# dmMaze/comic-text-detector

Measured on NVIDIA H100. Metric: pages/sec @1024x1024 synthetic, higher is better.
Workload: dtype fp16

## Files before the change

comic-text-detector_b200/csrc/refine_mk.cu:

```cuda
#include <cuda_runtime.h>
#include <limits.h>
#include <math.h>

#include "kernels.h"

namespace ctd {

namespace {

constexpr int kThreads = 256;
constexpr int kChunkPx = kRefineChunkPx;

struct WinState {
  int hist[4][256];
  unsigned long long xs[12];
  int lo[3], hi[3], otsu_t[3], ncol;
  int nproc, proc_kind[4], proc_neg[4];
  int area0, max1, cnt1, max2;
  int pad[2];
};

struct Ctx {
  const uint8_t* img_all;
  const uint8_t* mask_all;
  uint32_t* out_all;
  const RefineWin* wins;
  const RefineChunk* chunks;
  WinState* st;
  int mode;
  uint16_t* lab;
  uint16_t* roots;
  int* nroots;
  int* P;
  int* acc;
  uint8_t* grey;
  unsigned* cand;
  unsigned *pred, *merged, *tmp;
  size_t plane_words;
};
constexpr uint16_t kNoLabel = 0xffffu;
constexpr unsigned kMergeBit = 0x8000u;
static_assert(kChunkPx <= int(kMergeBit), "a chunk-local offset fits the 15 bits below kMergeBit");

struct View {
  RefineWin win;
  int w, rw, rh, y0, x0, rows, cols, i0, cnt, woff;
  const uint8_t* img;
  const uint8_t* mask;
};

__device__ __forceinline__ View view_of(const Ctx& c, int chunk) {
  View v;
  const RefineChunk ch = c.chunks[chunk];
  v.w = ch.win;
  v.win = c.wins[ch.win];
  v.rw = v.win.x2 - v.win.x1;
  v.rh = v.win.y2 - v.win.y1;
  v.y0 = ch.y0;
  v.x0 = ch.x0;
  v.rows = ch.rows;
  v.cols = min(v.rw - ch.x0, kChunkPx);
  v.i0 = ch.y0 * v.rw + ch.x0;
  v.cnt = ch.rows * v.cols;
  v.woff = ch.woff;
  v.img = c.img_all + size_t(v.win.page_off) * 3;
  v.mask = c.mask_all + size_t(v.win.page_off);
  return v;
}

__device__ __forceinline__ int chunk_start(int y, int x, int rw) {
  if (rw > kChunkPx) return y * rw + (x & ~(kChunkPx - 1));
  const int rows_per = refine_rows_per_chunk(rw);
  return (y / rows_per) * rows_per * rw;
}
static_assert((kChunkPx & (kChunkPx - 1)) == 0, "row segments start on multiples of kChunkPx");

__device__ __forceinline__ int uf_find(const int* L, int a) {
  int p = __ldcg(L + a);
  while (p != a) {
    a = p;
    p = __ldcg(L + a);
  }
  return a;
}
__device__ __forceinline__ int uf_find_compress(int* L, int a) {
  const int r = uf_find(L, a);
  while (a != r) {
    const int p = __ldcg(L + a);
    if (p <= r) break;
    atomicMin(&L[a], r);
    a = p;
  }
  return r;
}
__device__ __forceinline__ void uf_union(int* L, int a, int b) {
  bool done;
  do {
    a = uf_find(L, a);
    b = uf_find(L, b);
    if (a < b) {
      const int old = atomicMin(&L[b], a);
      done = old == b;
      b = old;
    } else if (b < a) {
      const int old = atomicMin(&L[a], b);
      done = old == a;
      a = old;
    } else {
      done = true;
    }
  } while (!done);
}

__device__ __forceinline__ void hist_add(int* hist, int bin) {
  const int b0 = __shfl_sync(0xffffffffu, bin, 0);
  if (__all_sync(0xffffffffu, bin == b0)) {
    if ((threadIdx.x & 31) == 0 && bin >= 0) atomicAdd(&hist[bin], 32);
    return;
  }
  if (bin >= 0) atomicAdd(&hist[bin], 1);
}

struct DivW { int d; float inv; bool fast; };
__device__ __forceinline__ DivW make_div(int d, int n) { return DivW{d, __frcp_rn(float(d)), n < (1 << 24)}; }
__device__ __forceinline__ void divmod(int i, const DivW& dv, int& q, int& r) {
  if (dv.fast) {
    q = __float2int_rz(__int2float_rn(i) * dv.inv);
    r = i - q * dv.d;
    if (r < 0) { --q; r += dv.d; } else if (r >= dv.d) { ++q; r -= dv.d; }
  } else {
    q = i / dv.d;
    r = i - q * dv.d;
  }
}

__device__ __forceinline__ unsigned tail_mask(int w, int cnt) {
  const int rem = cnt - 32 * w;
  return rem >= 32 ? 0xffffffffu : (1u << rem) - 1u;
}
__device__ __forceinline__ unsigned row_start_bits(int x0, int rw) {
  unsigned rs = 0u;
  for (int j = x0 == 0 ? 0 : rw - x0; j < 32; j += rw) rs |= 1u << j;
  return rs;
}
__device__ __forceinline__ int run_end(unsigned M, unsigned S, int sbit) {
  const unsigned stop = (~M | S) & (0xfffffffeu << sbit);
  return stop ? __ffs(stop) - 2 : 31;
}
__device__ __forceinline__ unsigned span_bits(int lo, int hi) {
  return (hi == 31 ? 0xffffffffu : ((2u << hi) - 1u)) & ~((1u << lo) - 1u);
}
__device__ __forceinline__ unsigned copied_word(const unsigned* src, int sb, int len, int db, int d) {
  const int r = 32 * d - db;
  if (r <= -32 || r >= len) return 0u;
  const int pos = sb + max(r, 0);
  unsigned o = __funnelshift_r(src[pos >> 5], src[(pos >> 5) + 1], pos & 31);
  if (len - max(r, 0) < 32) o &= (1u << (len - max(r, 0))) - 1u;
  return r < 0 ? o << -r : o;
}

constexpr int kU = 4;
constexpr int kExtWords = (3 * kChunkPx) / 32 + 4;
static_assert(3 * (kChunkPx + 2) / 32 + 2 < kExtWords, "a row segment's halo rectangle fits the shared bit masks");
struct Halo {
  int ystart, xs, ew, ext, off;
};
__device__ __forceinline__ Halo halo_of(const View& v) {
  Halo h;
  h.ystart = v.y0 > 0 ? v.y0 - 1 : 0;
  h.xs = v.x0 > 0 ? v.x0 - 1 : 0;
  h.ew = min(v.x0 + v.cols + 1, v.rw) - h.xs;
  h.ext = (min(v.y0 + v.rows + 1, v.rh) - h.ystart) * h.ew;
  h.off = (v.y0 - h.ystart) * h.ew + v.x0 - h.xs;
  return h;
}
__device__ __forceinline__ unsigned bits_from(const unsigned* M, int pos) {
  if (pos <= -32) return 0u;
  if (pos < 0) return M[0] << (-pos);
  const int w = pos >> 5, sft = pos & 31;
  return __funnelshift_r(M[w], M[w + 1], sft);
}
__device__ __forceinline__ void row_ends(int x, int rw, unsigned& rs, unsigned& re) {
  rs = row_start_bits(x, rw);
  int xe = x + 32;
  if (xe >= rw) xe %= rw;
  re = (rs >> 1) | (xe == 0 ? 0x80000000u : 0u);
}
__global__ void __launch_bounds__(kThreads) k_phase0(Ctx c) {
  __shared__ int sh[4][256];
  __shared__ unsigned N60[kExtWords], N127[kExtWords];
  __shared__ unsigned F127[kChunkPx / 32 + 1];
  const View v = view_of(c, blockIdx.x);
  for (int i = threadIdx.x; i < 1024; i += kThreads) (&sh[0][0])[i] = 0;
  for (int i = threadIdx.x; i < kExtWords; i += kThreads) { N60[i] = 0u; N127[i] = 0u; }
  __syncthreads();
  uint8_t* grey = c.grey + v.win.off;
  const Halo hl = halo_of(v);
  const DivW dv = make_div(hl.ew, 3 * (kChunkPx + 2) + 1);
  for (int e0 = 0; e0 < hl.ext; e0 += kThreads) {
    const int e = e0 + threadIdx.x;
    int mv = 255;
    if (e < hl.ext) {
      int ye, xe;
      divmod(e, dv, ye, xe);
      mv = v.mask[size_t(v.win.y1 + hl.ystart + ye) * v.win.pitch + v.win.x1 + hl.xs + xe];
    }
    const unsigned b60 = __ballot_sync(0xffffffffu, mv <= 60), b127 = __ballot_sync(0xffffffffu, mv <= 127);
    if ((threadIdx.x & 31) == 0 && e < hl.ext) { N60[e >> 5] = b60; N127[e >> 5] = b127; }
  }
  __syncthreads();
  const int ew = hl.ew;
  for (int w = threadIdx.x; w * 32 < v.cnt; w += kThreads) {
    const int p = w * 32 + hl.off;
    int ye, xe;
    divmod(p, dv, ye, xe);
    unsigned rs, re;
    row_ends(hl.xs + xe, v.rw, rs, re);
    const unsigned f60 = bits_from(N60, p) | bits_from(N60, p - ew) | bits_from(N60, p + ew) | (bits_from(N60, p - 1) & ~rs) |
                         (bits_from(N60, p + 1) & ~re);
    c.pred[v.woff + w] = ~f60 & tail_mask(w, v.cnt);
    c.merged[v.woff + w] = 0u;
    F127[w] = bits_from(N127, p) | bits_from(N127, p - ew) | bits_from(N127, p + ew) |
              ((bits_from(N127, p - 1) | bits_from(N127, p - ew - 1) | bits_from(N127, p + ew - 1)) & ~rs) |
              ((bits_from(N127, p + 1) | bits_from(N127, p - ew + 1) | bits_from(N127, p + ew + 1)) & ~re);
  }
  __syncthreads();
  const DivW dvw = make_div(v.rw, v.rw * v.rh);
  for (int k0 = 0; k0 < v.cnt; k0 += kThreads * kU) {
    int b[kU], g[kU], r[kU];
#pragma unroll
    for (int u = 0; u < kU; ++u) {
      const int k = k0 + u * kThreads + threadIdx.x;
      b[u] = -1; g[u] = -1; r[u] = -1;
      if (k < v.cnt) {
        int y, x;
        divmod(v.i0 + k, dvw, y, x);
        const size_t gp = size_t(v.win.y1 + y) * v.win.pitch + v.win.x1 + x;
        b[u] = v.img[gp * 3]; g[u] = v.img[gp * 3 + 1]; r[u] = v.img[gp * 3 + 2];
      }
    }
#pragma unroll
    for (int u = 0; u < kU; ++u) {
      const int k = k0 + u * kThreads + threadIdx.x;
      const bool in = k < v.cnt;
      int gr = 0;
      bool core = false;
      if (in) {
        const int i = v.i0 + k;
        gr = (b[u] * 1868 + g[u] * 9617 + r[u] * 4899 + 8192) >> 14;
        grey[i] = (uint8_t)gr;
        core = !((F127[k >> 5] >> (k & 31)) & 1u);
      }
      if (k0 + u * kThreads < v.cnt) {
        hist_add(sh[1], b[u]);
        hist_add(sh[2], g[u]);
        hist_add(sh[3], r[u]);
        hist_add(sh[0], core ? gr : -1);
      }
    }
  }
  __syncthreads();
  int* gh = &c.st[v.w].hist[0][0];
  for (int i = threadIdx.x; i < 1024; i += kThreads) {
    const int val = (&sh[0][0])[i];
    if (val) atomicAdd(&gh[i], val);
  }
}

constexpr int kDecideThreads = 64;
__global__ void __launch_bounds__(kDecideThreads) k_decide1(Ctx c) {
  __shared__ int cnt255[256];
  __shared__ int order[256];
  __shared__ double edges[256];
  __shared__ int s_first, s_last, s_total;
  __shared__ int hist_s[4][256];
  WinState& st = c.st[blockIdx.x];
  const RefineWin win = c.wins[blockIdx.x];
  const int n = (win.x2 - win.x1) * (win.y2 - win.y1);
  for (int i = threadIdx.x; i < 1024; i += kDecideThreads) (&hist_s[0][0])[i] = (&st.hist[0][0])[i];
  const int* hist_g = hist_s[0];
  for (int i = threadIdx.x; i < 256; i += kDecideThreads) cnt255[i] = 0;
  __syncthreads();
  if (threadIdx.x == 0) {
    int first = -1, last = -1, total = 0;
    for (int v = 0; v < 256; ++v)
      if (hist_g[v]) { if (first < 0) first = v; last = v; total += hist_g[v]; }
    s_first = first; s_last = last; s_total = total;
  }
  __syncthreads();
  {
    double fe, le;
    if (s_total == 0) { fe = 0.0; le = 1.0; }
    else if (s_first == s_last) { fe = s_first - 0.5; le = s_last + 0.5; }
    else { fe = s_first; le = s_last; }
    const double step = (le - fe) / 255.0;
    for (int i = threadIdx.x; i < 256; i += kDecideThreads) edges[i] = (i == 255) ? le : __dadd_rn(__dmul_rn((double)i, step), fe);
    __syncthreads();
    for (int v = threadIdx.x; v < 256; v += kDecideThreads) {
      if (!hist_g[v]) continue;
      const double a = (double)v;
      const double f = ((a - fe) / (le - fe)) * 255.0;
      int idx = (int)f;
      if (idx == 255) idx = 254;
      if (a < edges[idx]) --idx;
      if (a >= edges[idx + 1] && idx != 254) ++idx;
      atomicAdd(&cnt255[idx], hist_g[v]);
    }
  }
  __syncthreads();
  for (int b = threadIdx.x; b < 255; b += kDecideThreads) {
    int rank = 0;
    const int cb = cnt255[b];
    for (int q = 0; q < 255; ++q) rank += (cnt255[q] > cb) || (cnt255[q] == cb && q < b);
    order[rank] = b;
  }
  __syncthreads();
  if (threadIdx.x == 0) {
    double top[3];
    int nt = 1;
    top[0] = edges[order[0]];
    const double tol = (double)s_total * 0.001;
    for (int j = 1; j < 255; ++j) {
      const double col = edges[order[j]];
      double dmin = 1e300;
      for (int t = 0; t < nt; ++t) dmin = fmin(dmin, fabs(top[t] - col));
      if (dmin > 10.0) top[nt++] = col;
      if (nt >= 3 || (double)cnt255[order[j]] < tol) break;
    }
    st.ncol = nt;
    for (int t = 0; t < nt; ++t) {
      const double c_top = fmin(top[t] + 30.0, 255.0);
      const double c_bot = c_top - 60.0;
      st.lo[t] = (int)fmin(fmax(rint(c_bot), 0.0), 255.0);
      st.hi[t] = (int)fmin(fmax(rint(c_top), 0.0), 255.0);
    }
  }
  if (threadIdx.x >= 32 && threadIdx.x < 35) {
    const int* hh = hist_s[1 + threadIdx.x - 32];
    const double scale = 1.0 / (double)n;
    double mu = 0;
    for (int i = 0; i < 256; ++i) mu = __dadd_rn(mu, __dmul_rn((double)i, (double)hh[i]));
    mu = __dmul_rn(mu, scale);
    double mu1 = 0, q1 = 0, max_sigma = 0;
    int max_val = 0;
    for (int i = 0; i < 256; ++i) {
      const double p_i = __dmul_rn((double)hh[i], scale);
      mu1 = __dmul_rn(mu1, q1);
      q1 = __dadd_rn(q1, p_i);
      const double q2 = 1.0 - q1;
      if (fmin(q1, q2) < 1.1920929e-07 || fmax(q1, q2) > 1.0 - 1.1920929e-07) continue;
      mu1 = __ddiv_rn(__dadd_rn(mu1, __dmul_rn((double)i, p_i)), q1);
      const double mu2 = __ddiv_rn(__dsub_rn(mu, __dmul_rn(q1, mu1)), q2);
      const double dm = __dsub_rn(mu1, mu2);
      const double sigma = __dmul_rn(__dmul_rn(__dmul_rn(q1, q2), dm), dm);
      if (sigma > max_sigma) { max_sigma = sigma; max_val = i; }
    }
    st.otsu_t[threadIdx.x - 32] = max_val;
  }
}

__global__ void __launch_bounds__(kThreads) k_xor(Ctx c) {
  __shared__ unsigned long long sx[12];
  __shared__ unsigned Cw[6][kChunkPx / 32];
  const View v = view_of(c, blockIdx.x);
  const WinState& st = c.st[v.w];
  if (threadIdx.x < 12) sx[threadIdx.x] = 0ull;
  __syncthreads();
  const uint8_t* grey = c.grey + v.win.off;
  const int ncol = st.ncol;
  int lo[3], hi[3], ot[3];
#pragma unroll
  for (int k = 0; k < 3; ++k) { lo[k] = st.lo[k]; hi[k] = st.hi[k]; ot[k] = st.otsu_t[k]; }
  unsigned pos[6], npx = 0;
#pragma unroll
  for (int k = 0; k < 6; ++k) pos[k] = 0u;
  const DivW dv = make_div(v.rw, v.rw * v.rh);
  for (int k0 = 0; k0 < v.cnt; k0 += kThreads * kU) {
    int mk[kU], gr[kU], ch[kU][3];
#pragma unroll
    for (int u = 0; u < kU; ++u) {
      const int k = k0 + u * kThreads + threadIdx.x;
      mk[u] = -1; gr[u] = 0;
#pragma unroll
      for (int q = 0; q < 3; ++q) ch[u][q] = 0;
      if (k < v.cnt) {
        int y, x;
        divmod(v.i0 + k, dv, y, x);
        const size_t gp = size_t(v.win.y1 + y) * v.win.pitch + v.win.x1 + x;
        mk[u] = v.mask[gp];
        gr[u] = grey[v.i0 + k];
#pragma unroll
        for (int q = 0; q < 3; ++q) ch[u][q] = v.img[gp * 3 + q];
      }
    }
#pragma unroll
    for (int u = 0; u < kU; ++u) {
      const int kb = k0 + u * kThreads + (int(threadIdx.x) & ~31);
      if (kb >= v.cnt) continue;
      const bool in = mk[u] >= 0;
      npx += in;
#pragma unroll
      for (int k = 0; k < 3; ++k) {
        const bool t = in && gr[u] >= lo[k] && gr[u] <= hi[k];
        const bool t2 = in && ch[u][k] > ot[k];
        if (in) {
          pos[k] += (unsigned)((t ? 255 : 0) ^ mk[u]);
          pos[3 + k] += (unsigned)((t2 ? 255 : 0) ^ mk[u]);
        }
        const unsigned b = __ballot_sync(0xffffffffu, t), b2 = __ballot_sync(0xffffffffu, t2);
        if ((threadIdx.x & 31) == 0) { Cw[k][kb >> 5] = b; Cw[3 + k][kb >> 5] = b2; }
      }
    }
  }
#pragma unroll
  for (int k = 0; k < 6; ++k) {
    const bool used = k >= 3 || k < ncol;
    unsigned long long sp = used ? pos[k] : 0ull, sn = used ? 255ull * npx - pos[k] : 0ull;
    for (int o = 16; o > 0; o >>= 1) {
      sp += __shfl_down_sync(0xffffffffu, sp, o);
      sn += __shfl_down_sync(0xffffffffu, sn, o);
    }
    if ((threadIdx.x & 31) == 0) {
      if (sp) atomicAdd(&sx[2 * k], sp);
      if (sn) atomicAdd(&sx[2 * k + 1], sn);
    }
  }
  __syncthreads();
  if (threadIdx.x < 12 && sx[threadIdx.x]) atomicAdd(&c.st[v.w].xs[threadIdx.x], sx[threadIdx.x]);
  const int nw = (v.cnt + 31) >> 5;
  for (int k = 0; k < 6; ++k) {
    if (k < 3 && k >= ncol) continue;
    unsigned* cw = c.cand + k * c.plane_words + v.woff;
    for (int w = threadIdx.x; w < nw; w += kThreads) cw[w] = Cw[k][w];
  }
}

__global__ void k_decide2(Ctx c, int n_wins) {
  const int w = blockIdx.x * blockDim.x + threadIdx.x;
  if (w >= n_wins) return;
  WinState& st = c.st[w];
  const unsigned long long* xs = st.xs;
  unsigned long long best[4];
  int kind[4], neg[4], np_ = 0;
  for (int k = 0; k < st.ncol; ++k) {
    const bool ng = xs[2 * k + 1] < xs[2 * k];
    best[np_] = ng ? xs[2 * k + 1] : xs[2 * k];
    kind[np_] = k; neg[np_] = ng; ++np_;
  }
  int bc = 0, bneg = 0;
  unsigned long long bv = ~0ull;
  for (int ch = 0; ch < 3; ++ch) {
    const bool ng = xs[6 + 2 * ch + 1] < xs[6 + 2 * ch];
    const unsigned long long val = ng ? xs[6 + 2 * ch + 1] : xs[6 + 2 * ch];
    if (val < bv) { bv = val; bc = ch; bneg = ng; }
  }
  best[np_] = bv; kind[np_] = 3 + bc; neg[np_] = bneg; ++np_;
  for (int i = 1; i < np_; ++i) {
    const unsigned long long val = best[i];
    const int kk = kind[i], nn = neg[i];
    int j = i - 1;
    while (j >= 0 && best[j] > val) { best[j + 1] = best[j]; kind[j + 1] = kind[j]; neg[j + 1] = neg[j]; --j; }
    best[j + 1] = val; kind[j + 1] = kk; neg[j + 1] = nn;
  }
  for (int i = 0; i < np_; ++i) { st.proc_kind[i] = kind[i]; st.proc_neg[i] = neg[i]; }
  st.nproc = np_;
  st.area0 = 0; st.max1 = -1; st.cnt1 = 0; st.max2 = -1;
}

constexpr int kLabelThreads = 512;

struct Source { const unsigned* words; unsigned flip; };
__device__ __forceinline__ Source source_of(const Ctx& c, const WinState& st, const View& v, int round) {
  if (round == 4) return Source{c.merged + v.woff, 0xffffffffu};
  return Source{c.cand + size_t(st.proc_kind[round]) * c.plane_words + v.woff, st.proc_neg[round] ? 0xffffffffu : 0u};
}

__device__ void apply_merges(const Ctx& c, const View& v, int chunk, int round, unsigned* dec) {
  for (int i = threadIdx.x; i < kChunkPx / 32; i += blockDim.x) dec[i] = 0u;
  __syncthreads();
  const uint16_t* roots = c.roots + v.win.off + v.i0;
  const int nr = c.nroots[chunk];
  bool any = false;
  for (int j = threadIdx.x; j < nr; j += blockDim.x) {
    const unsigned e = roots[j];
    if (e & kMergeBit) { atomicOr(&dec[(e ^ kMergeBit) >> 5], 1u << (e & 31)); any = true; }
  }
  if (!__syncthreads_or(any)) return;
  const uint16_t* lab = c.lab + v.win.off + v.i0;
  const Source src = source_of(c, c.st[v.w], v, round);
  unsigned* merged = c.merged + v.woff;
  const DivW dv = make_div(v.rw, kChunkPx + 1);
  for (int hw0 = 0; hw0 * 16 < v.cnt; hw0 += blockDim.x) {
    const int hw = hw0 + threadIdx.x, w = hw >> 1;
    unsigned add = 0u;
    if (hw * 16 < v.cnt) {
      const unsigned M = (src.words[w] ^ src.flip) & tail_mask(w, v.cnt);
      if (M) {
        int yl, x0;
        divmod(w * 32, dv, yl, x0);
        const unsigned S = M & (~(M << 1) | row_start_bits(x0, v.rw));
        for (unsigned f = S & ((hw & 1) ? 0xffff0000u : 0x0000ffffu); f; f &= f - 1u) {
          const int sbit = __ffs(f) - 1;
          const unsigned l = lab[w * 32 + sbit];
          if ((dec[l >> 5] >> (l & 31)) & 1u) add |= span_bits(sbit, run_end(M, S, sbit));
        }
      }
    }
    add |= __shfl_xor_sync(0xffffffffu, add, 1);
    if (add && !(hw & 1)) merged[w] |= add;
  }
  __syncthreads();
}

__device__ __forceinline__ int suf_find(const int* L, int a) {
  int p = L[a];
  while (p != a) {
    a = p;
    p = L[a];
  }
  return a;
}
__device__ __forceinline__ int suf_find_halve(int* L, int a) {
  int p = L[a];
  while (p != a) {
    const int gp = L[p];
    if (gp != p) atomicMin(&L[a], gp);
    a = p;
    p = gp;
  }
  return a;
}
__device__ __forceinline__ void suf_union(int* L, int a, int b) {
  bool done;
  do {
    a = suf_find_halve(L, a);
    b = suf_find_halve(L, b);
    if (a < b) {
      const int old = atomicMin(&L[b], a);
      done = old == b;
      b = old;
    } else if (b < a) {
      const int old = atomicMin(&L[a], b);
      done = old == a;
      a = old;
    } else {
      done = true;
    }
  } while (!done);
}

#ifdef CTD_REFINE_PASS_CLOCKS
__device__ unsigned long long g_pass_clocks[5][8];
#define PASS_CLOCK_BEGIN() long long pass_t0 = clock64()
#define PASS_CLOCK(pass)                                                                        \
  do {                                                                                          \
    __syncthreads();                                                                            \
    if (threadIdx.x == 0) {                                                                     \
      const long long t = clock64();                                                            \
      atomicAdd(&g_pass_clocks[round][pass], (unsigned long long)(t - pass_t0));                \
      pass_t0 = t;                                                                              \
    }                                                                                           \
  } while (0)
#else
#define PASS_CLOCK_BEGIN()
#define PASS_CLOCK(pass)
#endif

__global__ void __launch_bounds__(kLabelThreads, 3) k_label_local(Ctx c, int round) {
  __shared__ int Ls[kChunkPx];
  __shared__ unsigned Mw[kChunkPx / 32 + 2];
  __shared__ unsigned Sw[kChunkPx / 32];
  __shared__ unsigned Gw[kChunkPx / 32];
  __shared__ unsigned Bw[kChunkPx / 32];
  __shared__ int s_fg, s_nroot;
  const View v = view_of(c, blockIdx.x);
  WinState& st = c.st[v.w];
  PASS_CLOCK_BEGIN();
  if (round >= 1 && round <= 3 && round - 1 < st.nproc) apply_merges(c, v, blockIdx.x, round - 1, Sw);
  if (round < 4 && round >= st.nproc) return;
  PASS_CLOCK(0);
  for (int i = threadIdx.x; i < kChunkPx / 32 + 2; i += kLabelThreads) Mw[i] = 0u;
  if (threadIdx.x == 0) { s_fg = 0; s_nroot = 0; }
  __syncthreads();
  uint16_t* lab = c.lab + v.win.off + v.i0;
  uint16_t* roots = c.roots + v.win.off + v.i0;
  int* P = c.P + v.win.off;
  int* acc = c.acc + 4 * v.win.off;
  const int n = v.rw * v.rh;
  int* area = acc; int* gain = acc + n; int* loss = acc + 2 * n; int* maxi = acc + 3 * n;
  const DivW dv = make_div(v.rw, kChunkPx + 1);
  {
    const Source src = source_of(c, st, v, round);
    const unsigned* mgw = c.merged + v.woff;
    const unsigned* pdw = c.pred + v.woff;
    for (int hw = threadIdx.x; hw * 16 < v.cnt; hw += kLabelThreads) {
      const int w = hw >> 1;
      const unsigned M = (src.words[w] ^ src.flip) & tail_mask(w, v.cnt);
      int yl, x0;
      divmod(w * 32, dv, yl, x0);
      const unsigned S = M & (~(M << 1) | row_start_bits(x0, v.rw));
      if (!(hw & 1)) {
        const unsigned un = M & ~mgw[w], pd = pdw[w];
        Mw[w] = M; Sw[w] = S; Gw[w] = un & pd; Bw[w] = un & ~pd;
      }
      for (unsigned f = S & ((hw & 1) ? 0xffff0000u : 0x0000ffffu); f; f &= f - 1u) {
        const int k = w * 32 + __ffs(f) - 1;
        Ls[k] = k;
      }
    }
  }
  __syncthreads();
  PASS_CLOCK(1);
  auto start_of = [&](int pos) -> int {
    return (pos & ~31) + 31 - __clz(Sw[pos >> 5] & (0xffffffffu >> (31 - (pos & 31))));
  };
  auto bits_at = [&](int pos) -> unsigned {
    if (pos <= -32) return 0u;
    if (pos < 0) return Mw[0] << (-pos);
    const int w = pos >> 5, sft = pos & 31;
    return __funnelshift_r(Mw[w], Mw[w + 1], sft);
  };
  for (int hw = threadIdx.x; hw * 16 < v.cnt; hw += kLabelThreads) {
    const int w = hw >> 1;
    const unsigned half = (hw & 1) ? 0xffff0000u : 0x0000ffffu;
    const unsigned cur = Mw[w];
    if (!(cur & half)) continue;
    const int k0 = w * 32;
    int yl, x0;
    divmod(k0, dv, yl, x0);
    const unsigned rs = row_start_bits(x0, v.rw);
    int xe = x0 + 32;
    if (xe >= v.rw) xe %= v.rw;
    const unsigned re = (rs >> 1) | (xe == 0 ? 0x80000000u : 0u);
    const unsigned lft = bits_at(k0 - 1);
    if (!(hw & 1) && (cur & 1u) && !(rs & 1u) && (lft & 1u)) suf_union(Ls, k0, start_of(k0 - 1));
    if (k0 + 32 <= v.rw) continue;
    const unsigned vup = (k0 >= v.rw ? 0xffffffffu : (0xffffffffu << (v.rw - k0))) & half;
    const unsigned up = bits_at(k0 - v.rw), upl = bits_at(k0 - v.rw - 1), upr = bits_at(k0 - v.rw + 1);
    unsigned f = cur & up & vup & (rs | ~lft | ~upl);
    while (f) {
      const int j = __ffs(f) - 1;
      f &= f - 1u;
      suf_union(Ls, start_of(k0 + j), start_of(k0 + j - v.rw));
    }
    const unsigned nb = cur & ~up & vup;
    f = nb & upl & ~rs;
    while (f) {
      const int j = __ffs(f) - 1;
      f &= f - 1u;
      suf_union(Ls, start_of(k0 + j), start_of(k0 + j - v.rw - 1));
    }
    f = nb & upr & ~re;
    while (f) {
      const int j = __ffs(f) - 1;
      f &= f - 1u;
      suf_union(Ls, start_of(k0 + j), start_of(k0 + j - v.rw + 1));
    }
  }
  __syncthreads();
  PASS_CLOCK(3);
  int fgc = 0;
  for (int hw = threadIdx.x; hw * 16 < v.cnt; hw += kLabelThreads) {
    const unsigned half = (hw & 1) ? 0xffff0000u : 0x0000ffffu;
    unsigned f = Sw[hw >> 1] & half;
    fgc += __popc(Mw[hw >> 1] & half);
    const int k0 = (hw >> 1) * 32;
    while (f) {
      const int s0 = k0 + __ffs(f) - 1;
      f &= f - 1u;
      const int r = suf_find(Ls, s0);
      if (r != s0) {
        atomicMin(&Ls[s0], r);
      } else {
        const int gi = v.i0 + s0;
        area[gi] = 0; gain[gi] = 0; loss[gi] = 0; maxi[gi] = -1;
        P[gi] = gi;
        roots[atomicAdd(&s_nroot, 1)] = uint16_t(s0);
      }
    }
  }
  if (round == 4) {
    for (int o = 16; o > 0; o >>= 1) fgc += __shfl_down_sync(0xffffffffu, fgc, o);
    if ((threadIdx.x & 31) == 0 && fgc) atomicAdd(&s_fg, fgc);
  }
  __syncthreads();
  if (threadIdx.x == 0) {
    c.nroots[blockIdx.x] = s_nroot;
    const int a0 = v.cnt - s_fg;
    if (round == 4 && a0) atomicAdd(&st.area0, a0);
  }
  PASS_CLOCK(4);
  for (int k = threadIdx.x; k < v.cnt; k += kLabelThreads)
    lab[k] = ((Mw[k >> 5] >> (k & 31)) & 1u) ? uint16_t(Ls[start_of(k)]) : kNoLabel;
  PASS_CLOCK(5);
  for (int hw = threadIdx.x; hw * 16 < v.cnt; hw += kLabelThreads) {
    const int w = hw >> 1;
    const unsigned M = Mw[w], S = Sw[w];
    unsigned f = S & ((hw & 1) ? 0xffff0000u : 0x0000ffffu);
    if (!f) continue;
    const unsigned G = Gw[w], B = Bw[w];
    const int k0 = w * 32;
    while (f) {
      const int sbit = __ffs(f) - 1;
      f &= f - 1u;
      const int e = run_end(M, S, sbit);
      const unsigned rm = span_bits(sbit, e);
      const int gi = v.i0 + Ls[k0 + sbit];
      atomicAdd(&area[gi], __popc(rm));
      atomicMax(&maxi[gi], v.i0 + k0 + e);
      const int g_ = __popc(rm & G), l_ = __popc(rm & B);
      if (g_) atomicAdd(&gain[gi], g_);
      if (l_) atomicAdd(&loss[gi], l_);
    }
  }
  PASS_CLOCK(6);
}
constexpr int kBorderThreads = 256;
__global__ void __launch_bounds__(kBorderThreads) k_union_border(Ctx c, int round) {
  const View v = view_of(c, blockIdx.x);
  if (round < 4 && round >= c.st[v.w].nproc) return;
  if (v.i0 == 0) return;
  const uint16_t* lab = c.lab + v.win.off;
  int* P = c.P + v.win.off;
  auto root_at = [&](int y, int x) { const int i = y * v.rw + x; return chunk_start(y, x, v.rw) + lab[i]; };
  const int y = v.y0;
  if (v.x0 > 0 && threadIdx.x == 0 && lab[v.i0] != kNoLabel && lab[v.i0 - 1] != kNoLabel)
    uf_union(P, v.i0 + lab[v.i0], root_at(y, v.x0 - 1));
  if (y == 0) return;
  for (int k = threadIdx.x; k < v.cols; k += int(blockDim.x)) {
    const int i = v.i0 + k, x = v.x0 + k;
    if (lab[i] == kNoLabel) continue;
    const int up = i - v.rw;
    const int r = v.i0 + lab[i];
    if (lab[up] != kNoLabel) {
      const bool first = x == 0 || lab[i - 1] == kNoLabel || lab[up - 1] == kNoLabel;
      if (first) uf_union(P, r, root_at(y - 1, x));
    } else {
      if (x > 0 && lab[up - 1] != kNoLabel) uf_union(P, r, root_at(y - 1, x - 1));
      if (x + 1 < v.rw && lab[up + 1] != kNoLabel) uf_union(P, r, root_at(y - 1, x + 1));
    }
  }
}
__global__ void __launch_bounds__(kThreads) k_flat1(Ctx c, int round) {
  const View v = view_of(c, blockIdx.x);
  if (round < 4 && round >= c.st[v.w].nproc) return;
  const uint16_t* roots = c.roots + v.win.off + v.i0;
  const int nr = c.nroots[blockIdx.x];
  int* P = c.P + v.win.off;
  int* acc = c.acc + 4 * v.win.off;
  const int n = v.rw * v.rh;
  int* area = acc; int* gain = acc + n; int* loss = acc + 2 * n; int* maxi = acc + 3 * n;
  for (int j = threadIdx.x; j < nr; j += kThreads) {
    const int cr = v.i0 + roots[j];
    const int g = uf_find_compress(P, cr);
    if (g != cr) {
      atomicAdd(&area[g], area[cr]);
      atomicMax(&maxi[g], maxi[cr]);
      const int g_ = gain[cr], l_ = loss[cr];
      if (g_) atomicAdd(&gain[g], g_);
      if (l_) atomicAdd(&loss[g], l_);
    }
  }
}
__global__ void __launch_bounds__(kThreads) k_top_a(Ctx c) {
  const View v = view_of(c, blockIdx.x);
  WinState& st = c.st[v.w];
  const int* P = c.P + v.win.off;
  const int* area = c.acc + 4 * v.win.off;
  const uint16_t* roots = c.roots + v.win.off + v.i0;
  const int nr = c.nroots[blockIdx.x];
  int m = -1;
  for (int j = threadIdx.x; j < nr; j += kThreads) {
    const int i = v.i0 + roots[j];
    if (P[i] == i) m = max(m, area[i]);
  }
  if (v.i0 == 0 && threadIdx.x == 0) m = max(m, st.area0);
  for (int o = 16; o > 0; o >>= 1) m = max(m, __shfl_down_sync(0xffffffffu, m, o));
  if ((threadIdx.x & 31) == 0 && m >= 0) atomicMax(&st.max1, m);
}
__global__ void __launch_bounds__(kThreads) k_top_b(Ctx c) {
  const View v = view_of(c, blockIdx.x);
  WinState& st = c.st[v.w];
  const int* P = c.P + v.win.off;
  const int* area = c.acc + 4 * v.win.off;
  const uint16_t* roots = c.roots + v.win.off + v.i0;
  const int nr = c.nroots[blockIdx.x];
  const int m1 = st.max1;
  int m2 = -1, c1 = 0;
  auto push = [&](int a) { if (a == m1) ++c1; else m2 = max(m2, a); };
  for (int j = threadIdx.x; j < nr; j += kThreads) {
    const int i = v.i0 + roots[j];
    if (P[i] == i) push(area[i]);
  }
  if (v.i0 == 0 && threadIdx.x == 0) push(st.area0);
  for (int o = 16; o > 0; o >>= 1) {
    m2 = max(m2, __shfl_down_sync(0xffffffffu, m2, o));
    c1 += __shfl_down_sync(0xffffffffu, c1, o);
  }
  if ((threadIdx.x & 31) == 0) {
    if (c1) atomicAdd(&st.cnt1, c1);
    if (m2 >= 0) atomicMax(&st.max2, m2);
  }
}
__global__ void __launch_bounds__(kThreads) k_decide_roots(Ctx c, int round) {
  const View v = view_of(c, blockIdx.x);
  const WinState& st = c.st[v.w];
  if (round < 4 && round >= st.nproc) return;
  const int* P = c.P + v.win.off;
  const int* acc = c.acc + 4 * v.win.off;
  const int n = v.rw * v.rh;
  const int* area = acc; const int* gain = acc + n; const int* loss = acc + 2 * n; const int* maxi = acc + 3 * n;
  const int second = st.cnt1 >= 2 ? st.max1 : st.max2;
  const int thresh = second >= 0 ? second : st.max1;
  uint16_t* roots = c.roots + v.win.off + v.i0;
  const int nr = c.nroots[blockIdx.x];
  for (int j = threadIdx.x; j < nr; j += kThreads) {
    const int cl = roots[j];
    const int g = P[v.i0 + cl];
    const int a = area[g];
    bool ok;
    if (round < 4) {
      const int mx = maxi[g];
      ok = !(a == 1 || (a == 2 && (mx == g + 1 || mx == g + v.rw)));
    } else {
      ok = a < thresh;
    }
    if (ok && gain[g] > loss[g]) roots[j] = uint16_t(cl | kMergeBit);
  }
}
__global__ void __launch_bounds__(kThreads) k_merge(Ctx c, int round) {
  __shared__ unsigned dec[kChunkPx / 32];
  const View v = view_of(c, blockIdx.x);
  if (round >= c.st[v.w].nproc) return;
  apply_merges(c, v, blockIdx.x, round, dec);
}

__global__ void __launch_bounds__(kThreads) k_dilate(Ctx c) {
  __shared__ unsigned Mw[kExtWords];
  const View v = view_of(c, blockIdx.x);
  for (int i = threadIdx.x; i < kExtWords; i += kThreads) Mw[i] = 0u;
  __syncthreads();
  const Halo hl = halo_of(v);
  const int ew = hl.ew;
  const DivW dv = make_div(ew, 3 * (kChunkPx + 2) + 1);
  const bool seg = v.rw > kChunkPx;
  const int nseg = (v.rw + kChunkPx - 1) / kChunkPx;
  const int rows_up = seg ? 1 : refine_rows_per_chunk(v.rw);
  if (!seg) {
    const bool up = v.y0 > 0, down = v.y0 + v.rows < v.rh;
    const unsigned* mu = up ? c.merged + c.chunks[blockIdx.x - 1].woff : nullptr;
    const unsigned* md = down ? c.merged + c.chunks[blockIdx.x + 1].woff : nullptr;
    for (int d = threadIdx.x; d * 32 < hl.ext; d += kThreads) {
      unsigned m = copied_word(c.merged + v.woff, 0, v.cnt, hl.off, d);
      if (up) m |= copied_word(mu, (rows_up - 1) * v.rw, v.rw, 0, d);
      if (down) m |= copied_word(md, 0, v.rw, hl.off + v.cnt, d);
      Mw[d] = m;
    }
  }
  for (int e0 = 0; seg && e0 < hl.ext; e0 += kThreads) {
    const int e = e0 + threadIdx.x;
    bool bit = false;
    if (e < hl.ext) {
      int ye, xe;
      divmod(e, dv, ye, xe);
      const int y = hl.ystart + ye, x = hl.xs + xe;
      const int dy = y < v.y0 ? -1 : (y >= v.y0 + v.rows ? 1 : 0);
      int ch = int(blockIdx.x) + dy * (seg ? nseg : 1), k;
      if (seg) {
        ch += x / kChunkPx - v.x0 / kChunkPx;
        k = x % kChunkPx;
      } else {
        k = (dy < 0 ? rows_up - 1 : (dy > 0 ? 0 : y - v.y0)) * v.rw + x;
      }
      const int wo = ch == int(blockIdx.x) ? v.woff : c.chunks[ch].woff;
      bit = (c.merged[wo + (k >> 5)] >> (k & 31)) & 1u;
    }
    const unsigned m = __ballot_sync(0xffffffffu, bit);
    if ((threadIdx.x & 31) == 0 && e < hl.ext) Mw[e >> 5] = m;
  }
  __syncthreads();
  for (int w = threadIdx.x; w * 32 < v.cnt; w += kThreads) {
    const int p = w * 32 + hl.off;
    int ye, xe;
    divmod(p, dv, ye, xe);
    unsigned rs, re;
    row_ends(hl.xs + xe, v.rw, rs, re);
    unsigned o = bits_from(Mw, p) | bits_from(Mw, p - ew) | bits_from(Mw, p + ew);
    o |= (bits_from(Mw, p - 1) | bits_from(Mw, p - ew - 1) | bits_from(Mw, p + ew - 1)) & ~rs;
    o |= (bits_from(Mw, p + 1) | bits_from(Mw, p - ew + 1) | bits_from(Mw, p + ew + 1)) & ~re;
    c.tmp[v.woff + w] = o & tail_mask(w, v.cnt);
  }
}
__global__ void __launch_bounds__(kThreads) k_or(Ctx c) {
  __shared__ unsigned dec[kChunkPx / 32];
  const View v = view_of(c, blockIdx.x);
  apply_merges(c, v, blockIdx.x, 4, dec);
  const unsigned* merged = c.merged + v.woff;
  const DivW dv = make_div(v.rw, v.rw * v.rh);
  for (int k = threadIdx.x; k < v.cnt; k += kThreads) {
    if (!((merged[k >> 5] >> (k & 31)) & 1u)) continue;
    int y, x;
    divmod(v.i0 + k, dv, y, x);
    const size_t gp = size_t(v.win.page_off) + size_t(v.win.y1 + y) * v.win.pitch + v.win.x1 + x;
    atomicOr(&c.out_all[gp >> 2], 0xffu << (8 * (gp & 3)));
  }
}

}

#ifdef CTD_REFINE_PASS_CLOCKS
extern "C" __attribute__((visibility("default"))) int ctd_refine_pass_clocks(unsigned long long* out) {
  static const unsigned long long zero[5 * 8] = {};
  cudaError_t e = cudaMemcpyFromSymbol(out, g_pass_clocks, sizeof(zero));
  if (e == cudaSuccess) e = cudaMemcpyToSymbol(g_pass_clocks, zero, sizeof(zero));
  return int(e);
}
#endif

size_t refine_mk_state_bytes(int n_wins) { return (size_t(n_wins) * sizeof(WinState) + 255) / 256 * 256; }
static size_t plane_words(size_t total_px, size_t n_chunks) { return total_px / 32 + n_chunks + 1; }
size_t refine_scratch_bytes(size_t total_px, size_t n_chunks) {
  return total_px * (4 + 16 + 2 + 2 + 1) + n_chunks * 4 + 9 * 4 * plane_words(total_px, n_chunks) + 4096;
}

cudaError_t refine_mk_launch(const uint8_t* d_img, const uint8_t* d_mask, const RefineWin* d_wins, int n_wins,
                             const RefineChunk* d_chunks, int n_chunks, int n_multi_chunks, void* d_state, size_t total_px,
                             void* scratch, int refine_mode, uint8_t* d_out, cudaStream_t s) {
  if (n_wins <= 0 || n_chunks <= 0) return cudaSuccess;
  Ctx c;
  c.img_all = d_img; c.mask_all = d_mask; c.out_all = reinterpret_cast<uint32_t*>(d_out);
  c.wins = d_wins;
  c.chunks = d_chunks;
  c.st = static_cast<WinState*>(d_state);
  c.mode = refine_mode;
  char* p = static_cast<char*>(scratch);
  c.P = reinterpret_cast<int*>(p); p += total_px * 4;
  c.acc = reinterpret_cast<int*>(p); p += total_px * 16;
  c.lab = reinterpret_cast<uint16_t*>(p); p += total_px * 2;
  c.roots = reinterpret_cast<uint16_t*>(p); p += total_px * 2;
  c.nroots = reinterpret_cast<int*>(p); p += size_t(n_chunks) * 4;
  c.grey = reinterpret_cast<uint8_t*>(p); p += total_px;
  c.plane_words = plane_words(total_px, size_t(n_chunks));
  c.cand = reinterpret_cast<unsigned*>(p); p += 6 * 4 * c.plane_words;
  c.pred = reinterpret_cast<unsigned*>(p); p += 4 * c.plane_words;
  c.merged = reinterpret_cast<unsigned*>(p); p += 4 * c.plane_words;
  c.tmp = reinterpret_cast<unsigned*>(p);
  cudaError_t e = cudaMemsetAsync(d_state, 0, refine_mk_state_bytes(n_wins), s);
  if (e != cudaSuccess) return e;
  const unsigned g = unsigned(n_chunks);
  k_phase0<<<g, kThreads, 0, s>>>(c);
  k_decide1<<<unsigned(n_wins), kDecideThreads, 0, s>>>(c);
  k_xor<<<g, kThreads, 0, s>>>(c);
  k_decide2<<<unsigned((n_wins + 127) / 128), 128, 0, s>>>(c, n_wins);
  for (int round = 0; round < 5; ++round) {
    if (round == 4) k_merge<<<g, kThreads, 0, s>>>(c, 3);
    if (round == 4 && refine_mode == 0) {
      k_dilate<<<g, kThreads, 0, s>>>(c);
      unsigned* t = c.merged; c.merged = c.tmp; c.tmp = t;
    }
    k_label_local<<<g, kLabelThreads, 0, s>>>(c, round);
    if (n_multi_chunks > 0) {
      k_union_border<<<unsigned(n_multi_chunks), kBorderThreads, 0, s>>>(c, round);
      k_flat1<<<unsigned(n_multi_chunks), kThreads, 0, s>>>(c, round);
    }
    if (round == 4) {
      k_top_a<<<g, kThreads, 0, s>>>(c);
      k_top_b<<<g, kThreads, 0, s>>>(c);
    }
    k_decide_roots<<<g, kThreads, 0, s>>>(c, round);
  }
  k_or<<<g, kThreads, 0, s>>>(c);
  return cudaGetLastError();
}

}
```

Baseline: 1083.

## Link word-crossing horizontal runs via ballot scan; shrink label CTAs to raise occupancy

Horizontal run continuations across 32-bit word boundaries are no longer resolved with atomic union-find inside the neighbour pass. A dedicated one-thread-per-word pass builds a ballot bitmap of words that are a single continuing run and scans back to find the true run start, writing the parent label directly. The label kernel also drops to 256 threads with 6 CTAs per SM instead of 512x3, and optional instrumentation counts contacts per pass. The intent is to cut atomic contention and serial find chains on long runs, at the cost of an extra barrier-separated pass and tighter register limits.

Result: faster. 1135, median of 6 (+4.7%).

```diff
diff --git a/comic-text-detector_b200/csrc/refine_mk.cu b/comic-text-detector_b200/csrc/refine_mk.cu
--- a/comic-text-detector_b200/csrc/refine_mk.cu
+++ b/comic-text-detector_b200/csrc/refine_mk.cu
@@ -467,7 +467,8 @@
   st.area0 = 0; st.max1 = -1; st.cnt1 = 0; st.max2 = -1;
 }
 
-constexpr int kLabelThreads = 512;
+constexpr int kLabelThreads = 256;
+constexpr int kLabelCtasPerSm = 6;
 
 struct Source { const unsigned* words; unsigned flip; };
 __device__ __forceinline__ Source source_of(const Ctx& c, const WinState& st, const View& v, int round) {
@@ -551,6 +552,13 @@
 
 #ifdef CTD_REFINE_PASS_CLOCKS
 __device__ unsigned long long g_pass_clocks[5][8];
+__device__ unsigned long long g_pass_counts[5][2];
+#define PASS_COUNT(i, n)                                                                        \
+  do {                                                                                          \
+    const unsigned pc_ = __reduce_add_sync(0xffffffffu, unsigned(n));                           \
+    if ((threadIdx.x & 31) == 0 && pc_)                                                         \
+      atomicAdd(&g_pass_counts[round][i], (unsigned long long)pc_);                             \
+  } while (0)
 #define PASS_CLOCK_BEGIN() long long pass_t0 = clock64()
 #define PASS_CLOCK(pass)                                                                        \
   do {                                                                                          \
@@ -562,16 +570,18 @@
     }                                                                                           \
   } while (0)
 #else
+#define PASS_COUNT(i, n) (void)(n)
 #define PASS_CLOCK_BEGIN()
 #define PASS_CLOCK(pass)
 #endif
 
-__global__ void __launch_bounds__(kLabelThreads, 3) k_label_local(Ctx c, int round) {
+__global__ void __launch_bounds__(kLabelThreads, kLabelCtasPerSm) k_label_local(Ctx c, int round) {
   __shared__ int Ls[kChunkPx];
   __shared__ unsigned Mw[kChunkPx / 32 + 2];
   __shared__ unsigned Sw[kChunkPx / 32];
   __shared__ unsigned Gw[kChunkPx / 32];
   __shared__ unsigned Bw[kChunkPx / 32];
+  __shared__ unsigned Tw[kChunkPx / 32 / 32];
   __shared__ int s_fg, s_nroot;
   const View v = view_of(c, blockIdx.x);
   WinState& st = c.st[v.w];
@@ -610,6 +620,31 @@
     }
   }
   __syncthreads();
+  static_assert(kChunkPx / 32 <= kLabelThreads, "pass 1b: one thread per word");
+  {
+    const int w = threadIdx.x;
+    bool cont = false;
+    if (w > 0 && w * 32 < v.cnt && (Mw[w] & 1u) && (Mw[w - 1] >> 31)) {
+      int yl, x0;
+      divmod(w * 32, dv, yl, x0);
+      cont = x0 != 0;
+    }
+    const unsigned tb = __ballot_sync(0xffffffffu, cont && Sw[w] == 1u);
+    if ((threadIdx.x & 31) == 0 && threadIdx.x < kChunkPx / 32) Tw[threadIdx.x >> 5] = tb;
+    __syncthreads();
+    if (cont) {
+      int u = w - 1;
+      unsigned t = ~Tw[u >> 5] & (0xffffffffu >> (31 - (u & 31)));
+      while (!t) {
+        u = (u & ~31) - 1;
+        t = ~Tw[u >> 5];
+      }
+      u = (u & ~31) + 31 - __clz(t);
+      Ls[w * 32] = u * 32 + 31 - __clz(Sw[u]);
+    }
+    PASS_COUNT(0, cont);
+  }
+  __syncthreads();
   PASS_CLOCK(1);
   auto start_of = [&](int pos) -> int {
     return (pos & ~31) + 31 - __clz(Sw[pos >> 5] & (0xffffffffu >> (31 - (pos & 31))));
@@ -620,6 +655,7 @@
     const int w = pos >> 5, sft = pos & 31;
     return __funnelshift_r(Mw[w], Mw[w + 1], sft);
   };
+  unsigned n_contacts = 0;
   for (int hw = threadIdx.x; hw * 16 < v.cnt; hw += kLabelThreads) {
     const int w = hw >> 1;
     const unsigned half = (hw & 1) ? 0xffff0000u : 0x0000ffffu;
@@ -633,11 +669,11 @@
     if (xe >= v.rw) xe %= v.rw;
     const unsigned re = (rs >> 1) | (xe == 0 ? 0x80000000u : 0u);
     const unsigned lft = bits_at(k0 - 1);
-    if (!(hw & 1) && (cur & 1u) && !(rs & 1u) && (lft & 1u)) suf_union(Ls, k0, start_of(k0 - 1));
     if (k0 + 32 <= v.rw) continue;
     const unsigned vup = (k0 >= v.rw ? 0xffffffffu : (0xffffffffu << (v.rw - k0))) & half;
     const unsigned up = bits_at(k0 - v.rw), upl = bits_at(k0 - v.rw - 1), upr = bits_at(k0 - v.rw + 1);
     unsigned f = cur & up & vup & (rs | ~lft | ~upl);
+    n_contacts += __popc(f) + __popc(cur & ~up & vup & upl & ~rs) + __popc(cur & ~up & vup & upr & ~re);
     while (f) {
       const int j = __ffs(f) - 1;
       f &= f - 1u;
@@ -657,6 +693,7 @@
       suf_union(Ls, start_of(k0 + j), start_of(k0 + j - v.rw + 1));
     }
   }
+  PASS_COUNT(1, n_contacts);
   __syncthreads();
   PASS_CLOCK(3);
   int fgc = 0;
@@ -911,8 +948,10 @@
 #ifdef CTD_REFINE_PASS_CLOCKS
 extern "C" __attribute__((visibility("default"))) int ctd_refine_pass_clocks(unsigned long long* out) {
   static const unsigned long long zero[5 * 8] = {};
-  cudaError_t e = cudaMemcpyFromSymbol(out, g_pass_clocks, sizeof(zero));
-  if (e == cudaSuccess) e = cudaMemcpyToSymbol(g_pass_clocks, zero, sizeof(zero));
+  cudaError_t e = cudaMemcpyFromSymbol(out, g_pass_clocks, sizeof(g_pass_clocks));
+  if (e == cudaSuccess) e = cudaMemcpyFromSymbol(out + 5 * 8, g_pass_counts, sizeof(g_pass_counts));
+  if (e == cudaSuccess) e = cudaMemcpyToSymbol(g_pass_clocks, zero, sizeof(g_pass_clocks));
+  if (e == cudaSuccess) e = cudaMemcpyToSymbol(g_pass_counts, zero, sizeof(g_pass_counts));
   return int(e);
 }
 #endif
```
